# baldhat/yolov10-3D

Hardware: AMD Instinct MI355X
Metric: train_images_per_sec (higher is better)
Workload: dtype bf16

## Files before the change

### include/y3d.h

```cpp
#ifndef Y3D_H
#define Y3D_H
#include <stdint.h>

#ifdef __cplusplus
extern "C" {
#endif

enum { Y3D_F32 = 0, Y3D_BF16 = 1 };
enum { Y3D_OK = 0, Y3D_ERR_INVALID = -1, Y3D_ERR_HIP = -2 };

const char* y3d_last_error(void);
int y3d_abi_version(void);
int y3d_device_info(char* name, int name_len, int* compute_units, int* lds_bytes, int* clock_khz);

int y3d_pack_weight_fwd(int dtype, const float* w_oihw, void* out, int Cout, int Cin_g, int Cin_g_pad, int kh, int kw, void* stream);
int y3d_pack_weight_dgrad(int dtype, const float* w_oihw, void* out, int Cout, int Cin_g, int groups, int kh, int kw, void* stream);
int y3d_mt_pack_weights(int dtype, const int64_t* desc, const int* chunk_tensor, const int* chunk_off, int nchunks, int chunk, void* stream);
int y3d_mt_fp8w_quantize(const int64_t* desc, const int* row_begin, int ntensors, int nrows, void* stream);
int y3d_fp8w_dequantize(const uint8_t* codes, const float* scale, float* w, int rows, int K, void* stream);
int y3d_fp8_quantize_act(const void* x, int64_t xsw, int64_t M, int C, uint8_t* q, uint8_t* s, void* stream);
int y3d_fp8_pack_weight_fwd(const uint8_t* codes, const float* scale, int rows, int Cg, uint8_t* wq, uint8_t* ws, void* stream);
int y3d_conv3x3_fp8_ok(int B, int H, int W, int Cin, int Cout, int groups);
int y3d_conv3x3_fp8_stat_rows(int B, int H, int W);
int y3d_fp8_scale_pitch(int C);
int y3d_conv3x3_fp8_fwd(const uint8_t* xq, const uint8_t* xs, int B, int H, int W, int Cin, const uint8_t* wq, const uint8_t* ws, void* y, int64_t ysw,
                        int Cout, int groups, float* stat_partials, const float* scale, const float* shift, int act, void* stream);
int y3d_fp8_quantize_grad(const void* dy, int64_t sw, const float* scale, int64_t M, int C, uint8_t* q, uint8_t* s, void* stream);
int y3d_fp8_pack_weight_dgrad(const uint8_t* codes, int Cout, int Cin, int groups, int lo, int hi, uint8_t* wq, uint8_t* ws, void* stream);
int y3d_conv3x3_fp8_dgrad_ok(int B, int H, int W, int Cin, int Cout, int groups);
int y3d_conv3x3_fp8_dgrad(const uint8_t* dyq, const uint8_t* dys, int64_t qsw, int spitch, int lo, int hi, int B, int H, int W, const uint8_t* wq, const uint8_t* ws,
                          void* dx, int64_t dxsw, int Cin, int groups, void* stream);
int y3d_conv_kpad(int dtype, int k_total);
int y3d_conv_stat_blocks(int B, int Ho, int Wo);
int y3d_conv2d_stat_rows(int dtype, int B, int H, int W, int Cin, int Cout, int groups, int kh, int kw, int stride, int pad);
enum { Y3D_OP_FWD = 0, Y3D_OP_BWD_DATA = 1, Y3D_OP_BWD_WEIGHT = 2 };
enum { Y3D_EPI_RAW = 0, Y3D_EPI_PARTIALS = 1, Y3D_EPI_AFFINE = 2, Y3D_EPI_AFFINE_RES = 3, Y3D_EPI_BIAS = 4 };
enum {
  Y3D_ROUTE_GENERIC = 0,
  Y3D_ROUTE_STREAM1X1 = 1,
  Y3D_ROUTE_SMALL = 2,
  Y3D_ROUTE_SMALL_S2 = 3,
  Y3D_ROUTE_S2_DGRAD = 4,
  Y3D_ROUTE_TILE8 = 5,
  Y3D_ROUTE_TILE16 = 6,
  Y3D_ROUTE_WIDE3_8 = 7,
  Y3D_ROUTE_WIDE3_16 = 8,
  Y3D_ROUTE_FLAT = 9,
  Y3D_ROUTE_WGRAD_SMALL = 10,
  Y3D_ROUTE_WGRAD_TILE = 11,
  Y3D_ROUTE_WGRAD_STREAM1X1 = 12
};
int y3d_conv2d_route(int dtype, int op, int epi, int B, int H, int W, int Cin, int Cout, int groups, int kh, int kw, int stride, int pad);
int y3d_conv2d_fwd(int dtype, const void* x, int64_t xsb, int64_t xsh, int64_t xsw, int B, int H, int W, int Cin,
                   const void* w_packed, const float* bias, void* y, int64_t ysw, int Ho, int Wo, int Cout, int groups,
                   int kh, int kw, int stride, int pad, float* stat_partials, void* stream);
int y3d_conv2d_fwd_affine(int dtype, const void* x, int64_t xsb, int64_t xsh, int64_t xsw, int B, int H, int W, int Cin,
                          const void* w_packed, const float* scale, const float* shift, int act, void* y, int64_t ysw, int Ho, int Wo,
                          int Cout, int groups, int kh, int kw, int stride, int pad, void* stream);
int y3d_conv2d_fwd_affine_res_ok(int dtype, int B, int H, int W, int Cin, int Cout, int groups, int kh, int kw, int stride, int pad);
int y3d_conv2d_fwd_affine_res(int dtype, const void* x, int64_t xsb, int64_t xsh, int64_t xsw, int B, int H, int W, int Cin,
                              const void* w_packed, const float* scale, const float* shift, int act, const void* res, int64_t rsw, void* y,
                              int64_t ysw, int Ho, int Wo, int Cout, int groups, int kh, int kw, int stride, int pad, void* stream);
int y3d_conv2d_bwd_data(int dtype, const void* dy, int64_t dsb, int64_t dsh, int64_t dsw, int B, int Ho, int Wo, int Cout,
                        const void* w_packed_dgrad, void* dx, int64_t xsw, int H, int W, int Cin, int groups, int kh, int kw,
                        int stride, int pad, void* stream);
int y3d_conv2d_wgrad_splits(int dtype, int B, int Ho, int Wo, int Cout, int Cin_g, int groups, int kh, int kw);
int y3d_conv2d_wgrad_plan(int dtype, int B, int H, int W, int Cin, int Cout, int groups, int kh, int kw, int stride, int pad);
int y3d_set_tile_kernels(int enable);
int y3d_set_stream1x1(int enable);
int y3d_get_stream1x1(void);
int y3d_get_tile_kernels(void);
int y3d_set_bn_wide_slabs(int enable);
int y3d_conv2d_bwd_weight(int dtype, const void* x, int64_t xsb, int64_t xsh, int64_t xsw, int B, int H, int W, int Cin,
                          int Cin_real, const void* dy, int64_t dsw, int Ho, int Wo, int Cout, int groups, int kh, int kw,
                          int stride, int pad, float* slab, int nsplit, float* grad_oihw, int accumulate, void* stream);
int y3d_wgrad_fold(const float* slab, int nsplit, int Cout, int taps, int Cin_g, int Cin_g_real, float* grad_oihw, int accumulate,
                   void* stream);

int y3d_dw_blocks(int64_t M);
int y3d_dw_wgrad_blocks(int64_t M);
int y3d_dw_pack_weight(const float* w_oihw, float* out_taps_c, int C, int kh, int kw, void* stream);
int y3d_dwconv2d_fwd(int dtype, const void* x, int64_t xsb, int64_t xsh, int64_t xsw, int B, int H, int W, int C,
                     const float* w_packed, void* y, int64_t ysw, int Ho, int Wo, int kh, int kw, int stride, int pad,
                     float* stat_partials, void* stream);
int y3d_dwconv2d_fwd_affine(int dtype, const void* x, int64_t xsb, int64_t xsh, int64_t xsw, int B, int H, int W, int C,
                            const float* w_packed, const float* scale, const float* shift, int act, int res_mode, const void* res, int64_t rsw,
                            void* z, int64_t zsw, int Ho, int Wo, int kh, int kw, int stride, int pad, void* stream);
int y3d_dwconv2d_bwd_data(int dtype, const void* dy, int64_t dsb, int64_t dsh, int64_t dsw, int B, int Ho, int Wo, int C,
                          const float* w_packed, void* dx, int64_t xsw, int H, int W, int kh, int kw, int stride, int pad,
                          void* stream);
int y3d_dwconv2d_bwd_weight(int dtype, const void* x, int64_t xsb, int64_t xsh, int64_t xsw, int B, int H, int W, int C,
                            const void* dy, int64_t dsw, int Ho, int Wo, int kh, int kw, int stride, int pad, float* slab,
                            float* grad_oihw, int accumulate, void* stream);
int y3d_dw_wgrad_fold(const float* slab, int nblk, int C, int taps, float* grad_oihw, int accumulate, void* stream);

int y3d_bn_finalize(const float* partials, int nblk, int C, int64_t count, const float* gamma, const float* beta, float eps,
                    float momentum, float* running_mean, float* running_var, float* mean, float* invstd, float* scale,
                    float* shift, void* stream);
int y3d_bn_eval_scale(int C, const float* gamma, const float* beta, const float* running_mean, const float* running_var,
                      float eps, float* scale, float* shift, void* stream);
int y3d_bn_act_fwd(int dtype, const void* y, int64_t ysw, const float* scale, const float* shift, int act, int res_mode,
                   const void* res, int64_t rsw, void* z, int64_t zsw, int64_t P, int C, void* stream);
int y3d_bn_act_fwd_q(const void* y, int64_t ysw, const float* scale, const float* shift, int act, void* z, int64_t zsw, uint8_t* q, uint8_t* s,
                     int64_t P, int C, void* stream);
int y3d_bn_bwd_blocks(int64_t P, int C);
int y3d_bn_act_bwd_reduce(int dtype, const void* y, int64_t ysw, const void* dz, int64_t dsw, const void* res, int64_t rsw,
                          const float* scale, const float* shift, const float* mean, const float* invstd, int act,
                          int res_mode, float* partials, int64_t P, int C, void* stream);
int y3d_bn_bwd_finalize(const float* partials, int nblk, int C, int64_t count, float* dgamma, float* dbeta, int accumulate,
                        float* mean_g, float* mean_gx, void* stream);
int y3d_bn_act_bwd_apply(int dtype, const void* y, int64_t ysw, const void* dz, int64_t dsw, const void* res, int64_t rsw,
                         const float* scale, const float* shift, const float* mean, const float* invstd,
                         const float* mean_g, const float* mean_gx, int act, int res_mode, int train, void* dy, int64_t dysw,
                         void* dres, int64_t drsw, int64_t P, int C, void* stream);
int y3d_colsum_partials(int dtype, const void* x, int64_t xsw, float* partials, int64_t P, int C, void* stream);

int y3d_maxpool_fwd(int dtype, const void* x, int64_t xsb, int64_t xsh, int64_t xsw, void* y, int64_t ysw, uint8_t* argmax,
                    int B, int H, int W, int C, int k, void* stream);
int y3d_maxpool_bwd(int dtype, const void* dy, int64_t dsw, const uint8_t* argmax, void* dx, int64_t xsw, int B, int H, int W,
                    int C, int k, void* stream);
int y3d_upsample2x_fwd(int dtype, const void* x, int64_t xsb, int64_t xsh, int64_t xsw, void* y, int64_t ysw, int B, int H, int W,
                       int C, void* stream);
int y3d_upsample2x_bwd(int dtype, const void* dy, int64_t dsb, int64_t dsh, int64_t dsw, void* dx, int64_t xsw, int B, int H,
                       int W, int C, void* stream);
int y3d_copy2d(int dtype, const void* x, int64_t xsw, void* y, int64_t ysw, int64_t P, int C, void* stream);
int y3d_occupy_cus(int n, const int* flag, float* buf, int64_t nbuf, void* stream);
int y3d_add2d(int dtype, const void* a, int64_t asw, const void* b, int64_t bsw, void* y, int64_t ysw, int64_t P, int C, void* stream);
int y3d_nchw_to_nhwc(int dtype, const float* x_nchw, void* y_nhwc, int B, int C, int H, int W, int Cpad, void* stream);
int y3d_stem_im2col(int dtype, const float* x_nchw, void* out, int B, int H, int W, int Ho, int Wo, void* stream);
int y3d_stem_im2col_u8(int dtype, const uint8_t* x, int hwc, void* out, int B, int H, int W, int Ho, int Wo, void* stream);
int y3d_stem_conv_eval(const void* x, int in_mode, const float* wcol, const float* scale, const float* shift, int act, void* y, int64_t ysw,
                       int B, int H, int W, int Cout, void* stream);
int y3d_stem_conv_train_rows(int B, int H, int W);
int y3d_stem_conv_train(const void* x, int in_mode, const float* wcol, void* y, int64_t ysw, void* xcol, float* part, int B, int H, int W,
                        int Cout, void* stream);
int y3d_nhwc_to_nchw(int dtype, const void* x_nhwc, int64_t xsw, float* y_nchw, int B, int C, int H, int W, void* stream);
int y3d_proj_fwd(int dtype, const void* x, int64_t xsw, const float* w, const float* bias, void* y, int64_t ysw, int64_t P,
                 int Cin, int Cout, void* stream);
int y3d_proj_bwd_data(int dtype, const void* dy, int64_t dsw, const float* w, void* dx, int64_t xsw, int64_t P, int Cin, int Cout,
                      void* stream);
int y3d_proj_blocks(int64_t P);
int y3d_proj_bwd_weight(int dtype, const void* x, int64_t xsw, const void* dy, int64_t dsw, float* slab, float* bias_slab,
                        float* grad_w, float* grad_b, int accumulate, int64_t P, int Cin, int Cout, void* stream);
int y3d_slab_reduce(const float* slab, float* out, int nblk, int64_t n, int accumulate, void* stream);
int y3d_proj_group_fwd(int dtype, int nb, int cin, const void* x, int64_t xsw, const int* xoff, const float* const* w,
                       const float* const* b, const int* couts, void* y, int64_t ysw, int64_t P, void* stream);
int y3d_proj_group_bwd_data(int dtype, int nb, int cin, const void* dy, int64_t dsw, const int* xoff, const float* const* w,
                            const int* couts, void* dx, int64_t xsw, int64_t P, void* stream);
int y3d_proj_group_fwd_bn_mfma(int nb, int cin, const void* y_pre, int64_t ysw, const int* xoff, const float* const* w, const float* const* b,
                               const int* couts, const float* scale, const float* shift, int act, void* out, int64_t osw, int64_t P,
                               void* stream);
int y3d_proj_group_bwd_weight_bn_mfma_blocks(int64_t P);
int y3d_proj_group_bwd_weight_bn_mfma(int nb, int cin, const void* y_pre, int64_t ysw, const int* xoff, const void* dout, int64_t dsw,
                                      const int* couts, const float* scale, const float* shift, int act, float* slab, float* bslab,
                                      float* const* dw, float* const* db, int64_t P, void* stream);
int y3d_proj_group_bn_bwd_blocks(int64_t P);
int y3d_proj_group_bn_bwd(int mode, int nb, int cin, const void* y_pre, int64_t ysw, const int* xoff, const void* dout, int64_t dsw,
                          const float* const* w, const int* couts, const float* scale, const float* shift, const float* mean,
                          const float* invstd, const float* mean_g, const float* mean_gx, int act, float* partials, int nblk, void* dy,
                          int64_t dysw, int64_t P, int C, void* stream);
int y3d_proj_group_blocks(int64_t P);
int y3d_proj_group_fwd_bn(int dtype, int nb, int cin, const void* y_pre, int64_t xsw, const int* xoff, const float* const* w,
                          const float* const* b, const int* couts, const float* scale, const float* shift, int act, void* out,
                          int64_t ysw, int64_t P, void* stream);
int y3d_proj_group_bwd_weight_bn(int dtype, int nb, int cin, const void* y_pre, int64_t xsw, const int* xoff, const void* dy, int64_t dsw,
                                 const int* couts, const float* scale, const float* shift, int act, float* slab, float* bslab,
                                 float* const* dw, float* const* db, int64_t P, void* stream);
int y3d_proj_group_bwd_weight(int dtype, int nb, int cin, const void* x, int64_t xsw, const int* xoff, const void* dy, int64_t dsw,
                              const int* couts, float* slab, float* bslab, float* const* dw, float* const* db, int64_t P, void* stream);

int y3d_attn_fwd(int dtype, const void* qkv, int64_t qsw, void* out, int64_t osw, float* lse, int B, int N, int nh, int kd, int hd,
                 float scale, void* stream);
int y3d_attn_bwd(int dtype, const void* qkv, int64_t qsw, const void* out, int64_t osw, const void* dout, int64_t dsw,
                 const void* dv_extra, int64_t esw, const float* lse, float* delta, void* dqkv, int64_t gsw, int B, int N, int nh,
                 int kd, int hd, float scale, void* stream);

int y3d_tal3d_scratch_floats(int B, int n, int A, int topk);
int y3d_pad_targets(const float* rows, int nbox, int width, int B, int cap, float scale_x, float scale_y, float* out, int* n_used,
                    void* stream);
int y3d_tal3d_assign(int dtype, int nl, const void* const* maps, const int64_t* psw, const int* H, const int* W, const float* strides,
                     int B, int nc, const float* gt, int n, const float* calib, const float* mean_sizes, int topk, float alpha,
                     float beta, float gamma, int mode, float* scratch, uint8_t* fg_mask, int* target_gt_idx, float* target_scores, float* scal,
                     const int* n_used, void* stream);
int y3d_loss3d(int dtype, int nl, const void* const* maps, const int64_t* psw, void* const* grads, const int64_t* gsw, const int* H,
               const int* W, const float* strides, int B, int nc, const float* gt, int n, const uint8_t* fg_mask,
               const int* target_gt_idx, const float* target_scores, const float* scal, float w_loss2d, float w_cls, float w_depth,
               float w_offset3d, float w_size3d, float w_heading, float grad_scale, float* partials, float* items, void* stream);
int y3d_loss3d_weighted(int dtype, int nl, const void* const* maps, const int64_t* psw, void* const* grads, const int64_t* gsw, const int* H,
                        const int* W, const float* strides, int B, int nc, const float* gt, int n, const uint8_t* fg_mask,
                        const int* target_gt_idx, const float* target_scores, const float* scal, float w_loss2d, float w_cls, float w_depth,
                        float w_offset3d, float w_size3d, float w_heading, float grad_scale, float* partials, float* items,
                        const float* item_w, float* total, void* stream);
int y3d_htl_update(const float* items, float time_value, int stat_epochs, float* ring, int* count, float* init_diff, int* have_init,
                   float* weights, int* status, void* stream);

int y3d_distill_loss(int dtype, int nl, const void* const* embs, const int64_t* psw, const int* H, const int* W, int B, int C,
                     const void* teacher, int teacher_dtype, int th, int tw, int64_t tsb, int64_t tsc, int64_t tsh, int64_t tsw,
                     const float* gt, int n, const uint8_t* fg_mask, const int* target_gt_idx, const float* scal, const uint8_t* mixed,
                     int img_w, int img_h, float T, float weight, int criterion, int no_mixup, int cap, int* counts, int* idx,
                     void* rows, float* partials, float* loss, void* stream);
int y3d_distill_scatter(int dtype, const void* rows, const int* idx, const int* nrows, const float* scale, int cap, int C, void* grad,
                        int64_t sb, int64_t sh, int64_t sw, int a0, int H, int W, void* stream);

int y3d_tal2d_assign(int dtype, int nl, const void* const* maps, const int64_t* psw, const int* H, const int* W, const float* strides,
                     int B, int nc, const float* gt, int n, int topk, float alpha, float beta, float* scratch, uint8_t* fg_mask,
                     int* target_gt_idx, float* target_scores, float* scal, const int* n_used, void* stream);
int y3d_loss2d(int dtype, int nl, const void* const* maps, const int64_t* psw, void* const* grads, const int64_t* gsw, const int* H,
               const int* W, const float* strides, int B, int nc, const float* gt, int n, const uint8_t* fg_mask,
               const int* target_gt_idx, const float* target_scores, const float* scal, float w_box, float w_cls, float w_dfl,
               float grad_scale, float* partials, float* items, void* stream);
int y3d_tal2d_scratch_floats(int B, int n, int A, int topk);
int y3d_tal2d_assign_crowded(int dtype, int nl, const void* const* maps, const int64_t* psw, const int* H, const int* W, const float* strides,
                             int B, int nc, const float* gt, int n, int topk, float alpha, float beta, float* scratch, uint8_t* fg_mask,
                             int* target_gt_idx, float* target_scores, float* scal, const int* n_used, void* stream);

int y3d_topk_cells(int dtype, const void* cls, int64_t psw, int B, int HW, int nc, int K, int* out_idx, void* stream);
int y3d_patch_gather(int dtype, const void* x, int64_t xsb, int64_t xsh, int64_t xsw, const int* idx, void* out, int B, int H, int W,
                     int C, int K, int ps, void* stream);
int y3d_head3d_scatter(int dtype, const void* cls, int64_t csw, const void* reg, int64_t rsw, const int* idx, void* map, int B, int HW,
                       int nc, int no, int K, void* stream);
int y3d_head3d_decode(int dtype, int nl, const void* const* maps, const int* H, const int* W, const float* strides, int B, int nc,
                      float* y, void* stream);
int y3d_head2d_decode(int dtype, int nl, const void* const* maps, const int* H, const int* W, const float* strides, int B, int nc,
                      float* y, void* stream);
int y3d_v10_postprocess_scratch_floats(int B, int A, int nc, int max_det);
// ... 122 lines not shown
```

### yolov10-3d_amd/_lib.py

```python
from __future__ import annotations

import ctypes
import os
import re

_HERE = os.path.dirname(os.path.abspath(__file__))
LIB_PATH = os.path.join(_HERE, "liby3d_hip.so")
HEADER = os.path.join(os.path.dirname(_HERE), "include", "y3d.h")

F32, BF16 = 0, 1

_CT = {"int": ctypes.c_int, "int64_t": ctypes.c_int64, "float": ctypes.c_float, "double": ctypes.c_double}


class Y3DError(RuntimeError):
    pass


def parse_header(path: str = HEADER):
    src = open(path).read()
    src = re.sub(r"/\*.*?\*/", " ", src, flags=re.S)
    protos = {}
    for m in re.finditer(r"(const\s+char\s*\*|int)\s+(y3d_\w+)\s*\(([^;{]*?)\)\s*;", src, flags=re.S):
        ret, name, args = m.group(1), m.group(2), m.group(3).strip()
        argtypes = []
        if args and args != "void":
            for a in args.split(","):
                a = a.strip()
                if "*" in a:
                    argtypes.append(ctypes.c_void_p)
                else:
                    toks = a.split()
                    t = toks[1] if toks[0] == "const" else toks[0]
                    argtypes.append(_CT[t])
        protos[name] = (ctypes.c_char_p if "char" in ret else ctypes.c_int, argtypes)
    return protos


_PLAIN_INT = {"abi_version", "conv_kpad", "conv_stat_blocks", "conv2d_stat_rows", "conv2d_route", "conv2d_wgrad_splits", "conv2d_wgrad_plan", "set_tile_kernels", "set_stream1x1", "set_bn_wide_slabs", "get_stream1x1", "get_tile_kernels", "dw_blocks", "dw_wgrad_blocks", "bn_bwd_blocks", "proj_blocks", "proj_group_blocks", "proj_group_bn_bwd_blocks", "proj_group_bwd_weight_bn_mfma_blocks", "tal3d_scratch_floats", "tal2d_scratch_floats", "v10_postprocess_scratch_floats", "conv2d_fwd_affine_res_ok", "stem_conv_train_rows", "conv3x3_fp8_ok", "conv3x3_fp8_dgrad_ok", "conv3x3_fp8_stat_rows", "fp8_scale_pitch", "kitti_eval_max_boxes", "det_metrics_max_gts", "det_metrics_max_dets"}


class _Lib:
    def __init__(self):
        if not os.path.exists(LIB_PATH):
            raise Y3DError(
                f"{LIB_PATH} not found: build it with `python yolov10-3d_amd/csrc/build.py` "
                "(or __graft_entry__.build()). There is no CPU / PyTorch fallback for the HIP path.")
        self._dll = ctypes.CDLL(LIB_PATH)
        self.protos = parse_header()
        for name, (ret, argtypes) in self.protos.items():
            fn = getattr(self._dll, name)
            fn.restype = ret
            fn.argtypes = argtypes

    def last_error(self) -> str:
        return (self._dll.y3d_last_error() or b"").decode()

    def __getattr__(self, name):
        if name.startswith("_"):
            raise AttributeError(name)
        fn = getattr(self._dll, "y3d_" + name)
        ret = self.protos["y3d_" + name][0]
        if ret is not ctypes.c_int or name in _PLAIN_INT:
            setattr(self, name, fn)
            return fn

        def call(*a):
            rc = fn(*a)
            if rc != 0:
                raise Y3DError(f"y3d_{name} failed ({rc}): {self.last_error()}")
            return rc

        setattr(self, name, call)
        return call


_lib = None


def lib() -> _Lib:
    global _lib
    if _lib is None:
        _lib = _Lib()
    return _lib
```

### yolov10-3d_amd/csrc/proj_bn_mfma.hip

```cpp
#include "common.h"

namespace {

constexpr int PB_MAXB = 16;

struct PBP {
  const bf16_t* y;
  const bf16_t* dout;
  bf16_t* dy;
  float* part;
  const float* w[PB_MAXB];
  int xoff[PB_MAXB], ooff[PB_MAXB], cout[PB_MAXB];
  const float *scale, *shift, *mean, *invstd, *mg, *mgx;
  long ysw, dsw, dysw, P;
  int cin, C, act, px_per_block;
};

template <int MODE, int NT>
__global__ __launch_bounds__(256) void projg_bn_bwd_kernel(PBP p) {
  constexpr int CIN = NT * 16, LDW = CIN + 4;
  constexpr int CH = CIN / 8;
  constexpr int PPP = 64 / CH;
  constexpr int NPASS = 16 / PPP;
  static_assert(NPASS >= 1 && 64 % CH == 0 && 16 % PPP == 0, "cin must be 32, 64 or 128");
  extern __shared__ __attribute__((aligned(16))) float psm[];
  const int tid = threadIdx.x, lane = tid & 63, wave = tid >> 6;
  const int q = lane >> 4, lp = lane & 15;
  const int br = blockIdx.y, cout = p.cout[br];
  float* tile = psm + wave * 16 * LDW;

  bf16x8_t wf[NT];
  {
    const float* w = p.w[br];
#pragma unroll
    for (int t = 0; t < NT; ++t)
#pragma unroll
      for (int j = 0; j < 8; ++j) {
        const int o = 8 * q + j;
        wf[t][j] = (__bf16)(o < cout ? w[o * CIN + t * 16 + lp] : 0.f);
      }
  }
  const int cc = lane % CH, pr = lane / CH;
  const int c0 = p.xoff[br] + cc * 8;
  float sc[8], sf[8], mu[8], is[8], m1[8], m2[8], s1[8], s2[8];
#pragma unroll
  for (int j = 0; j < 8; ++j) {
    sc[j] = p.scale[c0 + j]; sf[j] = p.shift[c0 + j]; mu[j] = p.mean[c0 + j]; is[j] = p.invstd[c0 + j];
    if (MODE == 1) { m1[j] = p.mg[c0 + j]; m2[j] = p.mgx[c0 + j]; }
    s1[j] = 0.f; s2[j] = 0.f;
  }
  const long pbeg = (long)blockIdx.x * p.px_per_block;
  const long pend = pbeg + p.px_per_block < p.P ? pbeg + p.px_per_block : p.P;
  const bf16_t* dop = p.dout + p.ooff[br];
  for (long pb = pbeg; pb < pend; pb += 64) {
    const long p0 = pb + wave * 16;
    uint4 yv[NPASS];
#pragma unroll
    for (int s = 0; s < NPASS; ++s) {
      const long px = p0 + s * PPP + pr;
      yv[s] = px < pend ? *(const uint4*)(p.y + px * p.ysw + c0) : make_uint4(0, 0, 0, 0);
    }
    bf16x8_t a;
    {
      const long px = p0 + lp;
      const bool pok = px < pend;
#pragma unroll
      for (int j = 0; j < 8; ++j) {
        const int o = 8 * q + j;
        unsigned short raw = 0;
        if (pok && o < cout) raw = dop[px * p.dsw + o];
        a[j] = __builtin_bit_cast(__bf16, raw);
      }
    }
#pragma unroll
    for (int t = 0; t < NT; ++t) {
      const f32x4_t d = __builtin_amdgcn_mfma_f32_16x16x32_bf16(a, wf[t], (f32x4_t){0.f, 0.f, 0.f, 0.f}, 0, 0, 0);
#pragma unroll
      for (int r = 0; r < 4; ++r) tile[(4 * q + r) * LDW + t * 16 + lp] = d[r];
    }
    __syncthreads();
#pragma unroll
    for (int s = 0; s < NPASS; ++s) {
      const int pl = s * PPP + pr;
      const long px = p0 + pl;
      const float4 z0 = *(const float4*)(tile + pl * LDW + cc * 8), z1 = *(const float4*)(tile + pl * LDW + cc * 8 + 4);
      const float dz[8] = {z0.x, z0.y, z0.z, z0.w, z1.x, z1.y, z1.z, z1.w};
      float v[8], o[8];
      Chunk<bf16_t>::unpack(yv[s], v);
#pragma unroll
      for (int j = 0; j < 8; ++j) {
        float g = dz[j];
        if (p.act) g *= silu_grad_f(v[j] * sc[j] + sf[j]);
        const float xh = (v[j] - mu[j]) * is[j];
        if (MODE == 0) { s1[j] += g; s2[j] += g * (v[j] - mu[j]) * is[j]; }
        else o[j] = sc[j] * (g - m1[j] - xh * m2[j]);
      }
      if (MODE == 1 && px < pend) *(uint4*)(p.dy + px * p.dysw + c0) = Chunk<bf16_t>::pack(o);
    }
    __syncthreads();
  }
  if (MODE == 0) {
    float* red = psm;
#pragma unroll
    for (int j = 0; j < 8; ++j) {
      red[((wave * PPP + pr) * CIN + cc * 8 + j) * 2 + 0] = s1[j];
      red[((wave * PPP + pr) * CIN + cc * 8 + j) * 2 + 1] = s2[j];
    }
    __syncthreads();
    if (tid < CIN) {
      float a0 = 0.f, a1 = 0.f;
      for (int r = 0; r < 4 * PPP; ++r) { a0 += red[(r * CIN + tid) * 2]; a1 += red[(r * CIN + tid) * 2 + 1]; }
      float* dst = p.part + ((long)blockIdx.x * p.C + p.xoff[br] + tid) * 2;
      dst[0] = a0;
      dst[1] = a1;
    }
  }
}

struct PFP {
  const bf16_t* y;
  bf16_t* out;
  const float* w[PB_MAXB];
  const float* b[PB_MAXB];
  int xoff[PB_MAXB], ooff[PB_MAXB], cout[PB_MAXB];
  const float *scale, *shift;
  long ysw, osw, P;
  int act, px_per_block;
};

template <int NT>
__global__ __launch_bounds__(256) void projg_fwd_bn_mfma_kernel(PFP p) {
  constexpr int CIN = NT * 16, KS = CIN / 32;
  constexpr int LDB = CIN * 2 + 16;
  constexpr int CH = CIN / 8, PPP = 64 / CH, NPASS = 16 / PPP;
  extern __shared__ __attribute__((aligned(16))) float psm[];
  const int tid = threadIdx.x, lane = tid & 63, wave = tid >> 6;
  const int q = lane >> 4, lp = lane & 15;
  const int br = blockIdx.y, cout = p.cout[br];
  char* tile = (char*)psm + wave * 16 * LDB;
  bf16x8_t wf[2][KS];
  float bias[2];
  {
    const float* w = p.w[br];
#pragma unroll
    for (int n = 0; n < 2; ++n) {
      const int o = 16 * n + lp;
      bias[n] = o < cout ? p.b[br][o] : 0.f;
#pragma unroll
      for (int ks = 0; ks < KS; ++ks)
#pragma unroll
        for (int j = 0; j < 8; ++j) wf[n][ks][j] = (__bf16)(o < cout ? w[o * CIN + ks * 32 + 8 * q + j] : 0.f);
    }
  }
  const int cc = lane % CH, pr = lane / CH;
  const int c0 = p.xoff[br] + cc * 8;
  float sc[8], sf[8];
#pragma unroll
  for (int j = 0; j < 8; ++j) { sc[j] = p.scale[c0 + j]; sf[j] = p.shift[c0 + j]; }
  const long pbeg = (long)blockIdx.x * p.px_per_block;
  const long pend = pbeg + p.px_per_block < p.P ? pbeg + p.px_per_block : p.P;
  bf16_t* op = p.out + p.ooff[br];
  const bool two = cout > 16;
  for (long pb = pbeg; pb < pend; pb += 64) {
    const long p0 = pb + wave * 16;
    uint4 yv[NPASS];
#pragma unroll
    for (int s = 0; s < NPASS; ++s) {
      const long px = p0 + s * PPP + pr;
      yv[s] = px < pend ? *(const uint4*)(p.y + px * p.ysw + c0) : make_uint4(0, 0, 0, 0);
    }
#pragma unroll
    for (int s = 0; s < NPASS; ++s) {
      float v[8];
      Chunk<bf16_t>::unpack(yv[s], v);
#pragma unroll
      for (int j = 0; j < 8; ++j) {
        const float u = v[j] * sc[j] + sf[j];
        v[j] = p.act ? silu_f(u) : u;
      }
      *(uint4*)(tile + (s * PPP + pr) * LDB + cc * 16) = Chunk<bf16_t>::pack(v);
    }
    __syncthreads();
    f32x4_t acc0 = {0.f, 0.f, 0.f, 0.f}, acc1 = {0.f, 0.f, 0.f, 0.f};
#pragma unroll
    for (int ks = 0; ks < KS; ++ks) {
      const bf16x8_t a = __builtin_bit_cast(bf16x8_t, *(const uint4*)(tile + lp * LDB + (ks * 4 + q) * 16));
      acc0 = __builtin_amdgcn_mfma_f32_16x16x32_bf16(a, wf[0][ks], acc0, 0, 0, 0);
      if (two) acc1 = __builtin_amdgcn_mfma_f32_16x16x32_bf16(a, wf[1][ks], acc1, 0, 0, 0);
    }
#pragma unroll
    for (int r = 0; r < 4; ++r) {
      const long px = p0 + 4 * q + r;
      if (px < pend) {
        if (lp < cout) op[px * p.osw + lp] = f2bf(acc0[r] + bias[0]);
        if (two && 16 + lp < cout) op[px * p.osw + 16 + lp] = f2bf(acc1[r] + bias[1]);
      }
    }
    __syncthreads();
  }
}

struct PWP {
  const bf16_t* y;
  const bf16_t* dout;
  float* slab;
  float* bslab;
  float* dw[PB_MAXB];
  float* db[PB_MAXB];
  int xoff[PB_MAXB], ooff[PB_MAXB], cout[PB_MAXB];
  const float *scale, *shift;
  long ysw, dsw, P;
  int act, px_per_block, ctot;
};

template <int NT>
__global__ __launch_bounds__(256) void projg_bwd_weight_bn_mfma_kernel(PWP p) {
  constexpr int CIN = NT * 16;
  constexpr int LDB = CIN * 2 + 32;
  constexpr int CH = CIN / 8, PPP = 64 / CH, NPASS = 32 / PPP;
  extern __shared__ __attribute__((aligned(16))) float psm[];
  const int tid = threadIdx.x, lane = tid & 63, wave = tid >> 6;
  const int g = lane >> 4, lp = lane & 15;
  const int br = blockIdx.y, cout = p.cout[br];
  const bool two = cout > 16;
  char* tile = (char*)psm + wave * 32 * LDB;
  const int cc = lane % CH, pr = lane / CH;
  const int c0 = p.xoff[br] + cc * 8;
  float sc[8], sf[8];
#pragma unroll
  for (int j = 0; j < 8; ++j) { sc[j] = p.scale[c0 + j]; sf[j] = p.shift[c0 + j]; }
  f32x4_t acc[2][NT];
#pragma unroll
  for (int n = 0; n < 2; ++n)
#pragma unroll
    for (int t = 0; t < NT; ++t) acc[n][t] = (f32x4_t){0.f, 0.f, 0.f, 0.f};
  float bsum[2] = {0.f, 0.f};
  const long pbeg = (long)blockIdx.x * p.px_per_block;
  const long pend = pbeg + p.px_per_block < p.P ? pbeg + p.px_per_block : p.P;
  const bf16_t* dop = p.dout + p.ooff[br];
  const int trow = 4 * g + (lp >> 2), tcol = (lp & 3) * 4;
  for (long pb = pbeg; pb < pend; pb += 128) {
    const long p0 = pb + wave * 32;
    uint4 yv[NPASS];
#pragma unroll
    for (int s = 0; s < NPASS; ++s) {
      const long px = p0 + s * PPP + pr;
      yv[s] = px < pend ? *(const uint4*)(p.y + px * p.ysw + c0) : make_uint4(0, 0, 0, 0);
    }
    bf16x8_t a[2];
#pragma unroll
    for (int n = 0; n < 2; ++n)
#pragma unroll
      for (int j = 0; j < 8; ++j) {
        const long px = p0 + 16 * (j >> 2) + 4 * g + (j & 3);
        const int o = 16 * n + lp;
        unsigned short raw = 0;
        if ((n == 0 || two) && o < cout && px < pend) raw = dop[px * p.dsw + o];
        a[n][j] = __builtin_bit_cast(__bf16, raw);
        bsum[n] += bf2f(raw);
      }
#pragma unroll
    for (int s = 0; s < NPASS; ++s) {
      float v[8];
      Chunk<bf16_t>::unpack(yv[s], v);
#pragma unroll
      for (int j = 0; j < 8; ++j) {
        const float u = v[j] * sc[j] + sf[j];
        v[j] = p.act ? silu_f(u) : u;
      }
      *(uint4*)(tile + (s * PPP + pr) * LDB + cc * 16) = Chunk<bf16_t>::pack(v);
    }
    __syncthreads();
#pragma unroll
    for (int t = 0; t < NT; ++t) {
      const char* a0 = tile + trow * LDB + (t * 16 + tcol) * 2;
      const s16x4_t lo = __builtin_amdgcn_ds_read_tr16_b64_v4i16((s16x4_t __attribute__((address_space(3)))*)(a0));
      const s16x4_t hi = __builtin_amdgcn_ds_read_tr16_b64_v4i16((s16x4_t __attribute__((address_space(3)))*)(a0 + 16 * LDB));
      typedef __attribute__((ext_vector_type(8))) short s16x8_t;
      const bf16x8_t b = __builtin_bit_cast(bf16x8_t, (s16x8_t)__builtin_shufflevector(lo, hi, 0, 1, 2, 3, 4, 5, 6, 7));
      acc[0][t] = __builtin_amdgcn_mfma_f32_16x16x32_bf16(a[0], b, acc[0][t], 0, 0, 0);
      if (two) acc[1][t] = __builtin_amdgcn_mfma_f32_16x16x32_bf16(a[1], b, acc[1][t], 0, 0, 0);
    }
    __syncthreads();
  }
  float* red = psm;
  const int NO = two ? 2 : 1;
  for (int n = 0; n < NO; ++n)
#pragma unroll
    for (int t = 0; t < NT; ++t)
#pragma unroll
      for (int r = 0; r < 4; ++r) red[(wave * 32 + 16 * n + 4 * g + r) * CIN + t * 16 + lp] = (n == 0 ? acc[0][t][r] : acc[1][t][r]);
  __shared__ float bred[4][32];
#pragma unroll
  for (int n = 0; n < 2; ++n) {
    float v = bsum[n];
    v = lane_xor32_sum(lane_xor16_sum(v));
    if (g == 0) bred[wave][16 * n + lp] = v;
  }
  __syncthreads();
  for (int i = tid; i < cout * CIN; i += 256) {
    const int o = i / CIN, ch = i - o * CIN;
    p.slab[((long)blockIdx.x * p.ctot + p.ooff[br] + o) * CIN + ch] =
        red[(0 * 32 + o) * CIN + ch] + red[(1 * 32 + o) * CIN + ch] + red[(2 * 32 + o) * CIN + ch] + red[(3 * 32 + o) * CIN + ch];
  }
  if (tid < cout) p.bslab[(long)blockIdx.x * p.ctot + p.ooff[br] + tid] = bred[0][tid] + bred[1][tid] + bred[2][tid] + bred[3][tid];
}

__device__ __forceinline__ float slab_sum_in_order(const float* __restrict__ src, long pitch, int nblk) {
  float s = 0.f;
  int b = 0;
  for (; b + 8 <= nblk; b += 8) {
    float v[8];
#pragma unroll
    for (int j = 0; j < 8; ++j) v[j] = src[(long)(b + j) * pitch];
#pragma unroll
    for (int j = 0; j < 8; ++j) s += v[j];
  }
  for (; b < nblk; ++b) s += src[(long)b * pitch];
  return s;
}

__global__ void projg_wslab_reduce_kernel(PWP p, int nblk, int cin) {
  const int br = blockIdx.y, cout = p.cout[br];
  const int idx = blockIdx.x * blockDim.x + threadIdx.x;
  if (idx < cout * cin) p.dw[br][idx] = slab_sum_in_order(p.slab + (long)p.ooff[br] * cin + idx, (long)p.ctot * cin, nblk);
  if (idx < cout) p.db[br][idx] = slab_sum_in_order(p.bslab + p.ooff[br] + idx, p.ctot, nblk);
}

}

extern "C" {

int y3d_proj_group_bwd_weight_bn_mfma_blocks(int64_t P) {
  long n = (P + 1023) / 1024;
  return (int)(n < 1 ? 1 : (n > 64 ? 64 : n));
}

int y3d_proj_group_bwd_weight_bn_mfma(int nb, int cin, const void* y_pre, int64_t ysw, const int* xoff, const void* dout, int64_t dsw,
                                      const int* couts, const float* scale, const float* shift, int act, float* slab, float* bslab,
                                      float* const* dw, float* const* db, int64_t P, void* stream) {
  Y3D_CHECK(nb >= 1 && nb <= PB_MAXB && (cin == 64 || cin == 128), "proj_group_bwd_weight_bn_mfma: 1..16 branches of 64 or 128 channels");
  Y3D_CHECK(y_pre && dout && scale && shift && slab && bslab && dw && db && P >= 1 && ysw % 8 == 0 && ((uintptr_t)y_pre & 15) == 0,
            "proj_group_bwd_weight_bn_mfma: null / misaligned argument");
  PWP p;
  p.y = (const bf16_t*)y_pre; p.dout = (const bf16_t*)dout; p.slab = slab; p.bslab = bslab;
  int off = 0;
  for (int i = 0; i < nb; ++i) {
    Y3D_CHECK(couts[i] >= 1 && couts[i] <= 32 && xoff[i] % 8 == 0, "proj_group_bwd_weight_bn_mfma: cout in 1..32, channel slices 16-byte aligned");
    p.dw[i] = dw[i]; p.db[i] = db[i]; p.xoff[i] = xoff[i]; p.ooff[i] = off; p.cout[i] = couts[i];
    off += couts[i];
  }
  Y3D_CHECK(dsw >= off, "proj_group_bwd_weight_bn_mfma: dout pixel stride smaller than the projected channels");
  p.scale = scale; p.shift = shift; p.ysw = ysw; p.dsw = dsw; p.P = P; p.act = act; p.ctot = off;
  const int nrun = y3d_proj_group_bwd_weight_bn_mfma_blocks(P);
  p.px_per_block = (int)(((P + nrun - 1) / nrun + 127) / 128 * 128);
  hipStream_t st = (hipStream_t)stream;
  const size_t sm = (size_t)4 * 32 * cin * sizeof(float);
  static bool attr = false;
  if (!attr) {
    (void)hipFuncSetAttribute((const void*)projg_bwd_weight_bn_mfma_kernel<8>, hipFuncAttributeMaxDynamicSharedMemorySize, 4 * 32 * 128 * 4);
    (void)hipFuncSetAttribute((const void*)projg_bwd_weight_bn_mfma_kernel<4>, hipFuncAttributeMaxDynamicSharedMemorySize, 4 * 32 * 64 * 4);
    attr = true;
  }
  if (cin == 128) hipLaunchKernelGGL((projg_bwd_weight_bn_mfma_kernel<8>), dim3(nrun, nb), dim3(256), sm, st, p);
  else hipLaunchKernelGGL((projg_bwd_weight_bn_mfma_kernel<4>), dim3(nrun, nb), dim3(256), sm, st, p);
  hipLaunchKernelGGL(projg_wslab_reduce_kernel, dim3((32 * cin + 255) / 256, nb), dim3(256), 0, st, p, nrun, cin);
  Y3D_LAUNCH_CHECK();
  return Y3D_OK;
}

int y3d_proj_group_fwd_bn_mfma(int nb, int cin, const void* y_pre, int64_t ysw, const int* xoff, const float* const* w, const float* const* b,
                               const int* couts, const float* scale, const float* shift, int act, void* out, int64_t osw, int64_t P,
                               void* stream) {
  Y3D_CHECK(nb >= 1 && nb <= PB_MAXB && (cin == 64 || cin == 128), "proj_group_fwd_bn_mfma: 1..16 branches of 64 or 128 channels");
  Y3D_CHECK(y_pre && out && w && b && scale && shift && P >= 1 && ysw % 8 == 0 && ((uintptr_t)y_pre & 15) == 0, "proj_group_fwd_bn_mfma: null / misaligned argument");
  PFP p;
  p.y = (const bf16_t*)y_pre; p.out = (bf16_t*)out;
  int off = 0;
  for (int i = 0; i < nb; ++i) {
    Y3D_CHECK(couts[i] >= 1 && couts[i] <= 32 && xoff[i] % 8 == 0, "proj_group_fwd_bn_mfma: cout in 1..32, channel slices 16-byte aligned");
    p.w[i] = w[i]; p.b[i] = b[i]; p.xoff[i] = xoff[i]; p.ooff[i] = off; p.cout[i] = couts[i];
    off += couts[i];
  }
  Y3D_CHECK(osw >= off, "proj_group_fwd_bn_mfma: output pixel stride smaller than the projected channels");
  p.scale = scale; p.shift = shift; p.ysw = ysw; p.osw = osw; p.P = P; p.act = act;
  long nrun = (P + 63) / 64;
  if (nrun > 128) nrun = 128;
  p.px_per_block = (int)(((P + nrun - 1) / nrun + 63) / 64 * 64);
  dim3 grid((unsigned)nrun, nb);
  hipStream_t st = (hipStream_t)stream;
  if (cin == 128) hipLaunchKernelGGL((projg_fwd_bn_mfma_kernel<8>), grid, dim3(256), (size_t)4 * 16 * (128 * 2 + 16), st, p);
  else hipLaunchKernelGGL((projg_fwd_bn_mfma_kernel<4>), grid, dim3(256), (size_t)4 * 16 * (64 * 2 + 16), st, p);
  Y3D_LAUNCH_CHECK();
  return Y3D_OK;
}

int y3d_proj_group_bn_bwd_blocks(int64_t P) {
  long n = (P + 63) / 64;
  return (int)(n < 1 ? 1 : (n > 128 ? 128 : n));
}

int y3d_proj_group_bn_bwd(int mode, int nb, int cin, const void* y_pre, int64_t ysw, const int* xoff, const void* dout, int64_t dsw,
                          const float* const* w, const int* couts, const float* scale, const float* shift, const float* mean,
                          const float* invstd, const float* mean_g, const float* mean_gx, int act, float* partials, int nblk, void* dy,
                          int64_t dysw, int64_t P, int C, void* stream) {
  Y3D_CHECK(mode == 0 || mode == 1, "proj_group_bn_bwd: mode 0 (reduce) or 1 (apply)");
  Y3D_CHECK(nb >= 1 && nb <= PB_MAXB && (cin == 64 || cin == 128), "proj_group_bn_bwd: 1..16 branches of 64 or 128 channels");
  Y3D_CHECK(y_pre && dout && scale && shift && mean && invstd && P >= 1, "proj_group_bn_bwd: null argument");
  Y3D_CHECK(mode == 0 ? (partials != nullptr && nblk == y3d_proj_group_bn_bwd_blocks(P)) : (dy && mean_g && mean_gx && dysw >= cin),
            "proj_group_bn_bwd: partials / nblk (reduce) or dy / mean_g / mean_gx (apply) missing");
  Y3D_CHECK(ysw % 8 == 0 && ((uintptr_t)y_pre & 15) == 0 && (mode == 0 || (dysw % 8 == 0 && ((uintptr_t)dy & 15) == 0)), "proj_group_bn_bwd: 16-byte alignment");
  PBP p;
  p.y = (const bf16_t*)y_pre; p.dout = (const bf16_t*)dout; p.dy = (bf16_t*)dy; p.part = partials;
  int off = 0;
  for (int i = 0; i < nb; ++i) {
    Y3D_CHECK(couts[i] >= 1 && couts[i] <= 32 && xoff[i] % 8 == 0 && xoff[i] + cin <= C, "proj_group_bn_bwd: cout in 1..32, channel slices 16-byte aligned inside C");
    p.w[i] = w[i]; p.xoff[i] = xoff[i]; p.ooff[i] = off; p.cout[i] = couts[i];
    off += couts[i];
  }
  Y3D_CHECK(dsw >= off, "proj_group_bn_bwd: dout pixel stride smaller than the projected channels");
  p.scale = scale; p.shift = shift; p.mean = mean; p.invstd = invstd; p.mg = mean_g; p.mgx = mean_gx;
  p.ysw = ysw; p.dsw = dsw; p.dysw = dysw; p.P = P; p.cin = cin; p.C = C; p.act = act;
  const int nrun = y3d_proj_group_bn_bwd_blocks(P);
  p.px_per_block = (int)(((P + nrun - 1) / nrun + 63) / 64 * 64);
  dim3 grid(nrun, nb);
  hipStream_t st = (hipStream_t)stream;
  const size_t sm128 = (size_t)4 * 16 * (128 + 4) * sizeof(float), sm64 = (size_t)4 * 16 * (64 + 4) * sizeof(float);
  if (cin == 128) {
    if (mode == 0) hipLaunchKernelGGL((projg_bn_bwd_kernel<0, 8>), grid, dim3(256), sm128, st, p);
    else hipLaunchKernelGGL((projg_bn_bwd_kernel<1, 8>), grid, dim3(256), sm128, st, p);
  } else {
    if (mode == 0) hipLaunchKernelGGL((projg_bn_bwd_kernel<0, 4>), grid, dim3(256), sm64, st, p);
    else hipLaunchKernelGGL((projg_bn_bwd_kernel<1, 4>), grid, dim3(256), sm64, st, p);
  }
  Y3D_LAUNCH_CHECK();
  return Y3D_OK;
}

}
```

Before: 1425.

## Skip all-zero upstream-gradient pixel groups in projection BN backward kernels

Adds a pre-scan of the projected output gradient in each block that records, per 64-pixel group and per 16-pixel wave slice, whether any nonzero values exist. The BN-backward reduce pass and the fused weight-gradient kernel then skip loads, MFMAs and LDS work for slices whose gradient is entirely zero, which targets sparse head gradients (e.g. masked 3D regression losses). The scan adds an extra read of dout and two barriers per block, and it only pays off when gradients are actually sparse. The feature is enabled by default and can be turned off with a new runtime toggle.

Measured after the change: 1443 (median of 6 runs). 1.3% higher.

```diff
diff --git a/include/y3d.h b/include/y3d.h
--- a/include/y3d.h
+++ b/include/y3d.h
@@ -71,6 +71,7 @@
 int y3d_get_stream1x1(void);
 int y3d_get_tile_kernels(void);
 int y3d_set_bn_wide_slabs(int enable);
+int y3d_set_proj_zero_skip(int enable);
 int y3d_conv2d_bwd_weight(int dtype, const void* x, int64_t xsb, int64_t xsh, int64_t xsw, int B, int H, int W, int Cin,
                           int Cin_real, const void* dy, int64_t dsw, int Ho, int Wo, int Cout, int groups, int kh, int kw,
                           int stride, int pad, float* slab, int nsplit, float* grad_oihw, int accumulate, void* stream);
diff --git a/yolov10-3d_amd/_lib.py b/yolov10-3d_amd/_lib.py
--- a/yolov10-3d_amd/_lib.py
+++ b/yolov10-3d_amd/_lib.py
@@ -37,7 +37,7 @@
     return protos
 
 
-_PLAIN_INT = {"abi_version", "conv_kpad", "conv_stat_blocks", "conv2d_stat_rows", "conv2d_route", "conv2d_wgrad_splits", "conv2d_wgrad_plan", "set_tile_kernels", "set_stream1x1", "set_bn_wide_slabs", "get_stream1x1", "get_tile_kernels", "dw_blocks", "dw_wgrad_blocks", "bn_bwd_blocks", "proj_blocks", "proj_group_blocks", "proj_group_bn_bwd_blocks", "proj_group_bwd_weight_bn_mfma_blocks", "tal3d_scratch_floats", "tal2d_scratch_floats", "v10_postprocess_scratch_floats", "conv2d_fwd_affine_res_ok", "stem_conv_train_rows", "conv3x3_fp8_ok", "conv3x3_fp8_dgrad_ok", "conv3x3_fp8_stat_rows", "fp8_scale_pitch", "kitti_eval_max_boxes", "det_metrics_max_gts", "det_metrics_max_dets"}
+_PLAIN_INT = {"abi_version", "conv_kpad", "conv_stat_blocks", "conv2d_stat_rows", "conv2d_route", "conv2d_wgrad_splits", "conv2d_wgrad_plan", "set_tile_kernels", "set_stream1x1", "set_bn_wide_slabs", "set_proj_zero_skip", "get_stream1x1", "get_tile_kernels", "dw_blocks", "dw_wgrad_blocks", "bn_bwd_blocks", "proj_blocks", "proj_group_blocks", "proj_group_bn_bwd_blocks", "proj_group_bwd_weight_bn_mfma_blocks", "tal3d_scratch_floats", "tal2d_scratch_floats", "v10_postprocess_scratch_floats", "conv2d_fwd_affine_res_ok", "stem_conv_train_rows", "conv3x3_fp8_ok", "conv3x3_fp8_dgrad_ok", "conv3x3_fp8_stat_rows", "fp8_scale_pitch", "kitti_eval_max_boxes", "det_metrics_max_gts", "det_metrics_max_dets"}
 
 
 class _Lib:
diff --git a/yolov10-3d_amd/csrc/proj_bn_mfma.hip b/yolov10-3d_amd/csrc/proj_bn_mfma.hip
--- a/yolov10-3d_amd/csrc/proj_bn_mfma.hip
+++ b/yolov10-3d_amd/csrc/proj_bn_mfma.hip
@@ -3,6 +3,7 @@
 namespace {
 
 constexpr int PB_MAXB = 16;
+int g_proj_zero_skip = 1;
 
 struct PBP {
   const bf16_t* y;
@@ -13,8 +14,56 @@
   int xoff[PB_MAXB], ooff[PB_MAXB], cout[PB_MAXB];
   const float *scale, *shift, *mean, *invstd, *mg, *mgx;
   long ysw, dsw, dysw, P;
-  int cin, C, act, px_per_block;
+  int cin, C, act, px_per_block, zskip;
 };
+
+constexpr int PZ_MAXGRP = 1024;
+
+__device__ __forceinline__ void projg_scan_dout(const bf16_t* dop, long dsw, int cout, long pbeg, long pend, int first, int ngrp,
+                                                unsigned char* zact, int wave, int lane) {
+  constexpr int GB = 8;
+  for (int i0 = first + wave; i0 < ngrp; i0 += 4 * GB) {
+    unsigned m[GB];
+#pragma unroll
+    for (int k = 0; k < GB; ++k) m[k] = 0;
+    for (int o0 = 0, ow = 1; o0 < cout; o0 += ow, ow = 8) {
+      unsigned bits[GB];
+#pragma unroll
+      for (int k = 0; k < GB; ++k) {
+        const long px = pbeg + (long)(i0 + 4 * k) * 64 + lane;
+        bits[k] = 0;
+        if (i0 + 4 * k < ngrp && px < pend) {
+          const bf16_t* r = dop + px * dsw + o0;
+#pragma unroll
+          for (int j = 0; j < 8; ++j)
+            if (j < ow && o0 + j < cout) bits[k] |= r[j];
+        }
+      }
+      bool full = true;
+#pragma unroll
+      for (int k = 0; k < GB; ++k) {
+        const unsigned long long bm = __ballot(bits[k] != 0);
+        m[k] |= ((bm & 0xFFFFull) ? 1u : 0u) | ((bm & 0xFFFF0000ull) ? 2u : 0u) | ((bm & 0xFFFF00000000ull) ? 4u : 0u) |
+                ((bm & 0xFFFF000000000000ull) ? 8u : 0u);
+        full = full && (m[k] == 0xFu || i0 + 4 * k >= ngrp);
+      }
+      if (full) break;
+    }
+#pragma unroll
+    for (int k = 0; k < GB; ++k)
+      if (lane == 0 && i0 + 4 * k < ngrp) zact[i0 + 4 * k] = (unsigned char)m[k];
+  }
+}
+
+__device__ __forceinline__ int projg_scan_run(const bf16_t* dop, long dsw, int cout, long pbeg, long pend, int ngrp, unsigned char* zact,
+                                              int wave, int lane) {
+  if (wave == 0) projg_scan_dout(dop, dsw, cout, pbeg, pend, 0, 1, zact, 0, lane);
+  __syncthreads();
+  if (__builtin_amdgcn_readfirstlane((int)zact[0]) == 0xF) return 0;
+  projg_scan_dout(dop, dsw, cout, pbeg, pend, 1, ngrp, zact, wave, lane);
+  __syncthreads();
+  return ngrp;
+}
 
 template <int MODE, int NT>
 __global__ __launch_bounds__(256) void projg_bn_bwd_kernel(PBP p) {
@@ -26,7 +75,7 @@
   extern __shared__ __attribute__((aligned(16))) float psm[];
   const int tid = threadIdx.x, lane = tid & 63, wave = tid >> 6;
   const int q = lane >> 4, lp = lane & 15;
-  const int br = blockIdx.y, cout = p.cout[br];
+  const int br = blockIdx.y, run = blockIdx.x, cout = p.cout[br];
   float* tile = psm + wave * 16 * LDW;
 
   bf16x8_t wf[NT];
@@ -49,53 +98,65 @@
     if (MODE == 1) { m1[j] = p.mg[c0 + j]; m2[j] = p.mgx[c0 + j]; }
     s1[j] = 0.f; s2[j] = 0.f;
   }
-  const long pbeg = (long)blockIdx.x * p.px_per_block;
+  const long pbeg = (long)run * p.px_per_block;
   const long pend = pbeg + p.px_per_block < p.P ? pbeg + p.px_per_block : p.P;
   const bf16_t* dop = p.dout + p.ooff[br];
+  __shared__ unsigned char zact[PZ_MAXGRP];
+  const int nstep = pend > pbeg ? (int)((pend - pbeg + 63) >> 6) : 0;
+  int nscan = (MODE == 0 && p.zskip) ? (nstep < PZ_MAXGRP ? nstep : PZ_MAXGRP) : 0;
+  if (nscan) nscan = projg_scan_run(dop, p.dsw, cout, pbeg, pend, nscan, zact, __builtin_amdgcn_readfirstlane(wave), lane);
   for (long pb = pbeg; pb < pend; pb += 64) {
+    const int step = (int)((pb - pbeg) >> 6);
+    const unsigned m = step < nscan ? (unsigned)__builtin_amdgcn_readfirstlane((int)zact[step]) : 0xFu;
+    if (m == 0) continue;
+    const bool live = __builtin_amdgcn_readfirstlane((int)((m >> wave) & 1u)) != 0;
     const long p0 = pb + wave * 16;
     uint4 yv[NPASS];
-#pragma unroll
-    for (int s = 0; s < NPASS; ++s) {
-      const long px = p0 + s * PPP + pr;
-      yv[s] = px < pend ? *(const uint4*)(p.y + px * p.ysw + c0) : make_uint4(0, 0, 0, 0);
-    }
-    bf16x8_t a;
-    {
-      const long px = p0 + lp;
-      const bool pok = px < pend;
-#pragma unroll
-      for (int j = 0; j < 8; ++j) {
-        const int o = 8 * q + j;
-        unsigned short raw = 0;
-        if (pok && o < cout) raw = dop[px * p.dsw + o];
-        a[j] = __builtin_bit_cast(__bf16, raw);
-      }
-    }
-#pragma unroll
-    for (int t = 0; t < NT; ++t) {
-      const f32x4_t d = __builtin_amdgcn_mfma_f32_16x16x32_bf16(a, wf[t], (f32x4_t){0.f, 0.f, 0.f, 0.f}, 0, 0, 0);
-#pragma unroll
-      for (int r = 0; r < 4; ++r) tile[(4 * q + r) * LDW + t * 16 + lp] = d[r];
-    }
-    __syncthreads();
-#pragma unroll
-    for (int s = 0; s < NPASS; ++s) {
-      const int pl = s * PPP + pr;
-      const long px = p0 + pl;
-      const float4 z0 = *(const float4*)(tile + pl * LDW + cc * 8), z1 = *(const float4*)(tile + pl * LDW + cc * 8 + 4);
-      const float dz[8] = {z0.x, z0.y, z0.z, z0.w, z1.x, z1.y, z1.z, z1.w};
-      float v[8], o[8];
-      Chunk<bf16_t>::unpack(yv[s], v);
-#pragma unroll
-      for (int j = 0; j < 8; ++j) {
-        float g = dz[j];
-        if (p.act) g *= silu_grad_f(v[j] * sc[j] + sf[j]);
-        const float xh = (v[j] - mu[j]) * is[j];
-        if (MODE == 0) { s1[j] += g; s2[j] += g * (v[j] - mu[j]) * is[j]; }
-        else o[j] = sc[j] * (g - m1[j] - xh * m2[j]);
-      }
-      if (MODE == 1 && px < pend) *(uint4*)(p.dy + px * p.dysw + c0) = Chunk<bf16_t>::pack(o);
+    if (live) {
+#pragma unroll
+      for (int s = 0; s < NPASS; ++s) {
+        const long px = p0 + s * PPP + pr;
+        yv[s] = px < pend ? *(const uint4*)(p.y + px * p.ysw + c0) : make_uint4(0, 0, 0, 0);
+      }
+      bf16x8_t a;
+      {
+        const long px = p0 + lp;
+        const bool pok = px < pend;
+#pragma unroll
+        for (int j = 0; j < 8; ++j) {
+          const int o = 8 * q + j;
+          unsigned short raw = 0;
+          if (pok && o < cout) raw = dop[px * p.dsw + o];
+          a[j] = __builtin_bit_cast(__bf16, raw);
+        }
+      }
+#pragma unroll
+      for (int t = 0; t < NT; ++t) {
+        const f32x4_t d = __builtin_amdgcn_mfma_f32_16x16x32_bf16(a, wf[t], (f32x4_t){0.f, 0.f, 0.f, 0.f}, 0, 0, 0);
+#pragma unroll
+        for (int r = 0; r < 4; ++r) tile[(4 * q + r) * LDW + t * 16 + lp] = d[r];
+      }
+    }
+    __syncthreads();
+    if (live) {
+#pragma unroll
+      for (int s = 0; s < NPASS; ++s) {
+        const int pl = s * PPP + pr;
+        const long px = p0 + pl;
+        const float4 z0 = *(const float4*)(tile + pl * LDW + cc * 8), z1 = *(const float4*)(tile + pl * LDW + cc * 8 + 4);
+        const float dz[8] = {z0.x, z0.y, z0.z, z0.w, z1.x, z1.y, z1.z, z1.w};
+        float v[8], o[8];
+        Chunk<bf16_t>::unpack(yv[s], v);
+#pragma unroll
+        for (int j = 0; j < 8; ++j) {
+          float g = dz[j];
+          if (p.act) g *= silu_grad_f(v[j] * sc[j] + sf[j]);
+          const float xh = (v[j] - mu[j]) * is[j];
+          if (MODE == 0) { s1[j] += g; s2[j] += g * (v[j] - mu[j]) * is[j]; }
+          else o[j] = sc[j] * (g - m1[j] - xh * m2[j]);
+        }
+        if (MODE == 1 && px < pend) *(uint4*)(p.dy + px * p.dysw + c0) = Chunk<bf16_t>::pack(o);
+      }
     }
     __syncthreads();
   }
@@ -110,7 +171,7 @@
     if (tid < CIN) {
       float a0 = 0.f, a1 = 0.f;
       for (int r = 0; r < 4 * PPP; ++r) { a0 += red[(r * CIN + tid) * 2]; a1 += red[(r * CIN + tid) * 2 + 1]; }
-      float* dst = p.part + ((long)blockIdx.x * p.C + p.xoff[br] + tid) * 2;
+      float* dst = p.part + ((long)run * p.C + p.xoff[br] + tid) * 2;
       dst[0] = a0;
       dst[1] = a1;
     }
@@ -210,7 +271,7 @@
   int xoff[PB_MAXB], ooff[PB_MAXB], cout[PB_MAXB];
   const float *scale, *shift;
   long ysw, dsw, P;
-  int act, px_per_block, ctot;
+  int act, px_per_block, ctot, zskip;
 };
 
 template <int NT>
@@ -221,7 +282,7 @@
   extern __shared__ __attribute__((aligned(16))) float psm[];
   const int tid = threadIdx.x, lane = tid & 63, wave = tid >> 6;
   const int g = lane >> 4, lp = lane & 15;
-  const int br = blockIdx.y, cout = p.cout[br];
+  const int br = blockIdx.y, run = blockIdx.x, cout = p.cout[br];
   const bool two = cout > 16;
   char* tile = (char*)psm + wave * 32 * LDB;
   const int cc = lane % CH, pr = lane / CH;
@@ -235,51 +296,63 @@
 #pragma unroll
     for (int t = 0; t < NT; ++t) acc[n][t] = (f32x4_t){0.f, 0.f, 0.f, 0.f};
   float bsum[2] = {0.f, 0.f};
-  const long pbeg = (long)blockIdx.x * p.px_per_block;
+  const long pbeg = (long)run * p.px_per_block;
   const long pend = pbeg + p.px_per_block < p.P ? pbeg + p.px_per_block : p.P;
   const bf16_t* dop = p.dout + p.ooff[br];
   const int trow = 4 * g + (lp >> 2), tcol = (lp & 3) * 4;
+  __shared__ unsigned char zact[PZ_MAXGRP];
+  const int ngrp = pend > pbeg ? 2 * (int)((pend - pbeg + 127) >> 7) : 0;
+  int nscan = p.zskip ? (ngrp < PZ_MAXGRP ? ngrp : PZ_MAXGRP) : 0;
+  if (nscan) nscan = projg_scan_run(dop, p.dsw, cout, pbeg, pend, nscan, zact, __builtin_amdgcn_readfirstlane(wave), lane);
   for (long pb = pbeg; pb < pend; pb += 128) {
+    const int g0 = (int)((pb - pbeg) >> 6);
+    const unsigned m = g0 < nscan ? (unsigned)__builtin_amdgcn_readfirstlane((int)zact[g0] | ((int)zact[g0 + 1] << 4)) : 0xFFu;
+    if (m == 0) continue;
+    const bool live = __builtin_amdgcn_readfirstlane((int)((m >> (2 * wave)) & 3u)) != 0;
     const long p0 = pb + wave * 32;
-    uint4 yv[NPASS];
-#pragma unroll
-    for (int s = 0; s < NPASS; ++s) {
-      const long px = p0 + s * PPP + pr;
-      yv[s] = px < pend ? *(const uint4*)(p.y + px * p.ysw + c0) : make_uint4(0, 0, 0, 0);
-    }
     bf16x8_t a[2];
-#pragma unroll
-    for (int n = 0; n < 2; ++n)
-#pragma unroll
-      for (int j = 0; j < 8; ++j) {
-        const long px = p0 + 16 * (j >> 2) + 4 * g + (j & 3);
-        const int o = 16 * n + lp;
-        unsigned short raw = 0;
-        if ((n == 0 || two) && o < cout && px < pend) raw = dop[px * p.dsw + o];
-        a[n][j] = __builtin_bit_cast(__bf16, raw);
-        bsum[n] += bf2f(raw);
-      }
-#pragma unroll
-    for (int s = 0; s < NPASS; ++s) {
-      float v[8];
-      Chunk<bf16_t>::unpack(yv[s], v);
-#pragma unroll
-      for (int j = 0; j < 8; ++j) {
-        const float u = v[j] * sc[j] + sf[j];
-        v[j] = p.act ? silu_f(u) : u;
-      }
-      *(uint4*)(tile + (s * PPP + pr) * LDB + cc * 16) = Chunk<bf16_t>::pack(v);
-    }
-    __syncthreads();
-#pragma unroll
-    for (int t = 0; t < NT; ++t) {
-      const char* a0 = tile + trow * LDB + (t * 16 + tcol) * 2;
-      const s16x4_t lo = __builtin_amdgcn_ds_read_tr16_b64_v4i16((s16x4_t __attribute__((address_space(3)))*)(a0));
-      const s16x4_t hi = __builtin_amdgcn_ds_read_tr16_b64_v4i16((s16x4_t __attribute__((address_space(3)))*)(a0 + 16 * LDB));
-      typedef __attribute__((ext_vector_type(8))) short s16x8_t;
-      const bf16x8_t b = __builtin_bit_cast(bf16x8_t, (s16x8_t)__builtin_shufflevector(lo, hi, 0, 1, 2, 3, 4, 5, 6, 7));
-      acc[0][t] = __builtin_amdgcn_mfma_f32_16x16x32_bf16(a[0], b, acc[0][t], 0, 0, 0);
-      if (two) acc[1][t] = __builtin_amdgcn_mfma_f32_16x16x32_bf16(a[1], b, acc[1][t], 0, 0, 0);
+    if (live) {
+      uint4 yv[NPASS];
+#pragma unroll
+      for (int s = 0; s < NPASS; ++s) {
+        const long px = p0 + s * PPP + pr;
+        yv[s] = px < pend ? *(const uint4*)(p.y + px * p.ysw + c0) : make_uint4(0, 0, 0, 0);
+      }
+#pragma unroll
+      for (int n = 0; n < 2; ++n)
+#pragma unroll
+        for (int j = 0; j < 8; ++j) {
+          const long px = p0 + 16 * (j >> 2) + 4 * g + (j & 3);
+          const int o = 16 * n + lp;
+          unsigned short raw = 0;
+          if ((n == 0 || two) && o < cout && px < pend) raw = dop[px * p.dsw + o];
+          a[n][j] = __builtin_bit_cast(__bf16, raw);
+          bsum[n] += bf2f(raw);
+        }
+#pragma unroll
+      for (int s = 0; s < NPASS; ++s) {
+        float v[8];
+        Chunk<bf16_t>::unpack(yv[s], v);
+#pragma unroll
+        for (int j = 0; j < 8; ++j) {
+          const float u = v[j] * sc[j] + sf[j];
+          v[j] = p.act ? silu_f(u) : u;
+        }
+        *(uint4*)(tile + (s * PPP + pr) * LDB + cc * 16) = Chunk<bf16_t>::pack(v);
+      }
+    }
+    __syncthreads();
+    if (live) {
+#pragma unroll
+      for (int t = 0; t < NT; ++t) {
+        const char* a0 = tile + trow * LDB + (t * 16 + tcol) * 2;
+        const s16x4_t lo = __builtin_amdgcn_ds_read_tr16_b64_v4i16((s16x4_t __attribute__((address_space(3)))*)(a0));
+        const s16x4_t hi = __builtin_amdgcn_ds_read_tr16_b64_v4i16((s16x4_t __attribute__((address_space(3)))*)(a0 + 16 * LDB));
+        typedef __attribute__((ext_vector_type(8))) short s16x8_t;
+        const bf16x8_t b = __builtin_bit_cast(bf16x8_t, (s16x8_t)__builtin_shufflevector(lo, hi, 0, 1, 2, 3, 4, 5, 6, 7));
+        acc[0][t] = __builtin_amdgcn_mfma_f32_16x16x32_bf16(a[0], b, acc[0][t], 0, 0, 0);
+        if (two) acc[1][t] = __builtin_amdgcn_mfma_f32_16x16x32_bf16(a[1], b, acc[1][t], 0, 0, 0);
+      }
     }
     __syncthreads();
   }
@@ -300,10 +373,10 @@
   __syncthreads();
   for (int i = tid; i < cout * CIN; i += 256) {
     const int o = i / CIN, ch = i - o * CIN;
-    p.slab[((long)blockIdx.x * p.ctot + p.ooff[br] + o) * CIN + ch] =
+    p.slab[((long)run * p.ctot + p.ooff[br] + o) * CIN + ch] =
         red[(0 * 32 + o) * CIN + ch] + red[(1 * 32 + o) * CIN + ch] + red[(2 * 32 + o) * CIN + ch] + red[(3 * 32 + o) * CIN + ch];
   }
-  if (tid < cout) p.bslab[(long)blockIdx.x * p.ctot + p.ooff[br] + tid] = bred[0][tid] + bred[1][tid] + bred[2][tid] + bred[3][tid];
+  if (tid < cout) p.bslab[(long)run * p.ctot + p.ooff[br] + tid] = bred[0][tid] + bred[1][tid] + bred[2][tid] + bred[3][tid];
 }
 
 __device__ __forceinline__ float slab_sum_in_order(const float* __restrict__ src, long pitch, int nblk) {
@@ -330,6 +403,12 @@
 }
 
 extern "C" {
+
+int y3d_set_proj_zero_skip(int enable) {
+  const int old = g_proj_zero_skip;
+  g_proj_zero_skip = enable ? 1 : 0;
+  return old;
+}
 
 int y3d_proj_group_bwd_weight_bn_mfma_blocks(int64_t P) {
   long n = (P + 1023) / 1024;
@@ -351,7 +430,7 @@
     off += couts[i];
   }
   Y3D_CHECK(dsw >= off, "proj_group_bwd_weight_bn_mfma: dout pixel stride smaller than the projected channels");
-  p.scale = scale; p.shift = shift; p.ysw = ysw; p.dsw = dsw; p.P = P; p.act = act; p.ctot = off;
+  p.scale = scale; p.shift = shift; p.ysw = ysw; p.dsw = dsw; p.P = P; p.act = act; p.ctot = off; p.zskip = g_proj_zero_skip;
   const int nrun = y3d_proj_group_bwd_weight_bn_mfma_blocks(P);
   p.px_per_block = (int)(((P + nrun - 1) / nrun + 127) / 128 * 128);
   hipStream_t st = (hipStream_t)stream;
@@ -420,7 +499,7 @@
   }
   Y3D_CHECK(dsw >= off, "proj_group_bn_bwd: dout pixel stride smaller than the projected channels");
   p.scale = scale; p.shift = shift; p.mean = mean; p.invstd = invstd; p.mg = mean_g; p.mgx = mean_gx;
-  p.ysw = ysw; p.dsw = dsw; p.dysw = dysw; p.P = P; p.cin = cin; p.C = C; p.act = act;
+  p.ysw = ysw; p.dsw = dsw; p.dysw = dysw; p.P = P; p.cin = cin; p.C = C; p.act = act; p.zskip = g_proj_zero_skip;
   const int nrun = y3d_proj_group_bn_bwd_blocks(P);
   p.px_per_block = (int)(((P + nrun - 1) / nrun + 63) / 64 * 64);
   dim3 grid(nrun, nb);
```
